# XiangpengHao/pq-vector

Measured on AMD Instinct MI355X. Metric: topk_queries_per_s_k10, higher is better.
Workload: dtype f32

## Files before the change

pq-vector_amd/csrc/api.cpp:

```cpp
#include "../../include/pqv.h"

#include <hip/hip_runtime.h>
#include <time.h>
#include <unistd.h>

#include <algorithm>
#include <atomic>
#include <functional>
#include <system_error>
#include <thread>
#include <cmath>
#include <chrono>
#include <cstdio>
#include <cstdlib>
#include <cstring>
#include <condition_variable>
#include <memory>
#include <mutex>
#include <new>
#include <string>
#include <type_traits>
#include <unordered_map>
#include <unordered_set>
#include <vector>
// ... 271 lines not shown
    }
};

constexpr int PQV_LANES = 4;
struct Scratch {
    DevBuf s_probe_keys, s_probe_vals, s_probe, s_cand_base, s_ncand, s_part_keys, s_part_vals, s_queries, s_rows,
        s_dist, s_nfound, s_pair_u32, s_pairs, s_groups, s_quads, s_items, s_ticket, s_ticket2, s_cand_keys, s_cand_vals, s_cand_cnt, s_spilled,
        s_seed_ub, s_qblk, s_gthr, s_tie, s_replay, s_qnorm, s_qmax, s_thr_hist, s_thr_bins, s_qi8, s_qn2i, s_qres, s_qresu, s_pair_lb, s_part_flags, s_qpad, s_cand_lb, s_pendv, s_work, s_nwork, s_out,
        s_hit_cnt, s_hit_keys, s_hit_vals, s_alt_keys, s_alt_vals, s_rsegs, s_rout_off, s_rout_rows, s_rout_dist,
        s_pair_end, s_file_cnt,
        s_qcos,
        s_qkeys,
        s_qfilt_a, s_qfilt_b,
        s_part_grp, s_grp_out,
        s_g1_rows, s_g1_dist, s_g1_keys, s_g1_nfound, s_gset_keys, s_gset_slot, s_gpart_slot, s_gpart_cnt, s_grows_out,
        s_expand_cnt, s_expand_used;
    PinnedBuf h_io;
    hipEvent_t done = nullptr;
    hipStream_t stream = nullptr;
    bool used = false;
    hipStream_t side = nullptr;
    hipEvent_t ev_fork = nullptr, ev_join = nullptr;
    std::vector<const DevBuf *> bufs() const {
        return {&s_probe_keys, &s_probe_vals, &s_probe, &s_cand_base, &s_ncand, &s_part_keys, &s_part_vals, &s_queries, &s_rows,
                &s_dist, &s_nfound, &s_pair_u32, &s_pairs, &s_groups, &s_quads, &s_items, &s_ticket, &s_ticket2, &s_cand_keys, &s_cand_vals, &s_cand_cnt, &s_spilled,
                &s_seed_ub, &s_qblk, &s_gthr, &s_tie, &s_replay, &s_qnorm, &s_qmax, &s_thr_hist, &s_thr_bins, &s_qi8, &s_qn2i, &s_qres, &s_qresu, &s_pair_lb, &s_part_flags, &s_qpad, &s_cand_lb, &s_pendv, &s_work, &s_nwork, &s_out,
                &s_hit_cnt, &s_hit_keys, &s_hit_vals, &s_alt_keys, &s_alt_vals, &s_rsegs, &s_rout_off, &s_rout_rows, &s_rout_dist,
                &s_pair_end, &s_file_cnt, &s_qcos, &s_qkeys, &s_qfilt_a, &s_qfilt_b, &s_part_grp, &s_grp_out,
                &s_g1_rows, &s_g1_dist, &s_g1_keys, &s_g1_nfound, &s_gset_keys, &s_gset_slot, &s_gpart_slot, &s_gpart_cnt, &s_grows_out,
                &s_expand_cnt, &s_expand_used};
    }
    ~Scratch() {
        if (done) (void)hipEventDestroy(done);
        if (ev_fork) (void)hipEventDestroy(ev_fork);
        if (ev_join) (void)hipEventDestroy(ev_join);
        if (side) (void)hipStreamDestroy(side);
    }
};

struct pqv_searcher {
    int device = 0;
    uint64_t uid = 0;
    uint32_t dim = 0, n_clusters = 0;
    uint32_t sdim = 0;
    uint64_t n = 0;
    uint64_t max_list_len = 0;
    pqv_corpus *corpus = nullptr;
    std::vector<uint64_t> h_list_off;
    std::shared_ptr<ListRows> h_rows;
    DevBuf d_cent_t;
    uint32_t kc_pad = 0;
    DevBuf d_centroids, d_list_off, d_ids, d_mat_ivf, d_stats;
    mutable DevBuf d_row_norm2;
    const float *d_mat = nullptr;
    const uint32_t *d_row_of = nullptr;
    const uint32_t *d_final_ids = nullptr;
    bool images_only = false;
    hipStream_t stream = nullptr;
    mutable std::mutex mu;
    mutable Scratch lanes[PQV_LANES];
    mutable PinnedBuf h_wide_stats;
    mutable uint32_t lane_rr = 0;
    mutable DevBuf d_mat_blk_op[3], d_blk_off;
    mutable bool f16_ok = false;
    mutable float f16_scale = 1.0f;
    mutable bool norms_done = false;
// ... 10 lines not shown
        uint32_t cand_cap = 0;
        int screen_f16 = 1;
        int screen_i8 = 1;
        uint32_t seed_rows = 0;
        uint32_t wide_rows = 0;
        uint32_t tile_rows = 0;
        int running_thr = 1;
        int defer = 1;
        int quad_xcd = -1;
        int single_bucket = 1;
        int seed_refine = 1;
        int item_grid = 1;
        int chunk_major = 1;
        int wide_waves = 0;
        int probe_rows = 1;
        uint32_t quad_width = 0;
        uint32_t min_blocks = 0;
        int pair_prune = 1;
        int i8_form = 0;
        int xcd_items = 1;
        int pf96 = 1;
        int drain_min = 0;
        int fork_wide = 0;
        int wide_quads = 1;
        uint32_t wide_quad_rows = 0;
        int list_once = 0;
    };
    mutable Opts opt;
    uint32_t n_files = 0;
    std::vector<uint32_t> seg_off;
    std::vector<uint64_t> row_base;
    uint32_t seg_max_kc = 0;
    bool rr_cap = false;
    DevBuf d_seg_off, d_seg_off64;
    mutable pqv_counters_t counters{};
    mutable bool timing = false;
    mutable std::vector<hipEvent_t> ev;
    mutable std::unique_ptr<pqv_corpus> cos_corpus;
    mutable std::unique_ptr<pqv_searcher> cos;
    ~pqv_searcher();
};
pqv_searcher::~pqv_searcher() {
    for (auto e : ev) (void)hipEventDestroy(e);
    pool_put(device, stream);
}

static int lane_acquire(const pqv_searcher *s, hipStream_t stream, Scratch **out) {
    Scratch *sc = nullptr;
    for (auto &l : s->lanes) if (l.used && l.stream == stream) { sc = &l; break; }
    if (!sc) for (auto &l : s->lanes) if (!l.used) { sc = &l; break; }
    if (!sc) sc = &s->lanes[s->lane_rr++ % PQV_LANES];
    if (!sc->done) HIP_TRY(hipEventCreateWithFlags(&sc->done, hipEventDisableTiming));
    if (sc->used && sc->stream != stream) HIP_TRY(hipStreamWaitEvent(stream, sc->done, 0));
    sc->stream = stream; sc->used = true;
    *out = sc;
    return PQV_OK;
}
// ... 2556 lines not shown
    o.cand_cap = static_cast<uint32_t>(std::max<long long>(0, num("PQV_CAND_CAP", o.cand_cap)));
    o.screen_f16 = num("PQV_SCREEN_F16", o.screen_f16) != 0;
    o.screen_i8 = static_cast<int>(num("PQV_SCREEN_I8", o.screen_i8));
    o.seed_rows = static_cast<uint32_t>(num("PQV_SEED_ROWS", o.seed_rows));
    o.wide_rows = static_cast<uint32_t>(num("PQV_WIDE_ROWS", o.wide_rows));
    o.tile_rows = static_cast<uint32_t>(num("PQV_TILE_ROWS", o.tile_rows));
    o.running_thr = num("PQV_RUNNING_THR", o.running_thr) != 0;
    o.defer = static_cast<int>(num("PQV_DEFER", o.defer));
    o.quad_xcd = static_cast<int>(num("PQV_QUAD_XCD", o.quad_xcd));
    o.wide_waves = static_cast<int>(num("PQV_WIDE_WAVES", o.wide_waves));
    o.item_grid = static_cast<int>(num("PQV_ITEM_GRID", o.item_grid));
    o.chunk_major = static_cast<int>(num("PQV_CHUNK_MAJOR", o.chunk_major));
    o.seed_refine = static_cast<int>(num("PQV_SEED_REFINE", o.seed_refine));
    o.single_bucket = static_cast<int>(num("PQV_SINGLE_BUCKET", o.single_bucket));
    o.probe_rows = static_cast<int>(num("PQV_PROBE_ROWS", o.probe_rows));
    o.quad_width = static_cast<uint32_t>(num("PQV_QUAD_WIDTH", o.quad_width));
    o.min_blocks = static_cast<uint32_t>(num("PQV_MIN_BLOCKS", o.min_blocks));
    o.wide_quads = static_cast<int>(num("PQV_WIDE_QUADS", o.wide_quads));
    o.fork_wide = static_cast<int>(num("PQV_FORK_WIDE", o.fork_wide));
    o.drain_min = static_cast<int>(num("PQV_DRAIN_MIN", o.drain_min));
    o.pf96 = static_cast<int>(num("PQV_PF96", o.pf96));
    o.xcd_items = static_cast<int>(num("PQV_XCD_ITEMS", o.xcd_items));
    o.wide_quad_rows = static_cast<uint32_t>(num("PQV_WIDE_QUAD_ROWS", o.wide_quad_rows));
    o.list_once = static_cast<int>(num("PQV_LIST_ONCE", o.list_once));
    o.pair_prune = static_cast<int>(num("PQV_PAIR_PRUNE", o.pair_prune));
    o.i8_form = static_cast<int>(num("PQV_I8_FORM", o.i8_form));
}

bool wide_rows_nt(const pqv_searcher *s) {
    if (!s->h_wide_stats.p) return true;
// ... 135 lines not shown
        HIP_TRY(hipStreamSynchronize(stream));
    } else if (op == 1) {
        HIP_TRY(blk.alloc(tiles * 16 * s->sdim * 2));
        HIP_TRY(launch_block_rows_f16(s->d_mat, s->d_list_off.as<uint64_t>(), s->d_blk_off.as<uint64_t>(), kc,
                                      (s->max_list_len + 15) / 16, s->sdim, s->f16_scale, blk.p, stream, s->d_row_of));
    } else {
        HIP_TRY(blk.alloc(tiles * 16 * s->sdim * sizeof(float)));
        HIP_TRY(launch_block_rows(s->d_mat, s->d_list_off.as<uint64_t>(), s->d_blk_off.as<uint64_t>(), kc,
                                  (s->max_list_len + 15) / 16, s->sdim, blk.p, stream, s->d_row_of));
    }
    HIP_TRY(hipStreamSynchronize(stream));
    undo.done = true;
    return PQV_OK;
}

}

static int pqv_searcher_create_impl(const pqv_index *index, pqv_corpus *corpus, uint32_t flags,
                                   pqv_searcher **out) {
    if (!out) return fail(PQV_ERR_INVALID, "out must not be NULL");
    *out = nullptr;
    const auto t_enter = std::chrono::steady_clock::now();
    if (!index || !corpus) return fail(PQV_ERR_INVALID, "index/corpus must not be NULL");
    if (index->dim != corpus->dim)
        return fail(PQV_ERR_INVALID, "index dimension " + std::to_string(index->dim) +
                                         " does not match corpus dimension " + std::to_string(corpus->dim));
    if (index->permutation_of != 0 ? index->permutation_of != corpus->n : false)
        return fail(PQV_ERR_INVALID, "index row id out of range for this corpus");
    uint64_t known_bound = 0;
    if (index->permutation_of == 0 && !(index->known_row_bound(&known_bound) && known_bound <= corpus->n)) {
// ... 40 lines not shown
    mark("validation + host copies");
    S_TRY(pool_get(s->device, &s->stream));
    mark("stream");
    S_TRY(s->d_centroids.alloc(index->centroids.size() * sizeof(float)));
    S_TRY(s->d_list_off.alloc(index->list_off.size() * sizeof(uint64_t)));
    S_TRY(s->d_ids.alloc(std::max<size_t>(1, s->n) * sizeof(uint32_t)));
    mark("allocations");
    S_TRY(hipMemcpyAsync(s->d_centroids.p, index->centroids.data(), index->centroids.size() * sizeof(float),
                         hipMemcpyHostToDevice, s->stream));
    S_TRY(hipMemcpyAsync(s->d_list_off.p, index->list_off.data(), index->list_off.size() * sizeof(uint64_t),
                         hipMemcpyHostToDevice, s->stream));
    if ((s->dim % 4) == 0 && s->n_clusters) {
        s->kc_pad = (s->n_clusters + 255) / 256 * 256;
        S_TRY(s->d_cent_t.alloc(static_cast<size_t>(s->kc_pad) * s->dim * sizeof(float)));
        S_TRY(pqv::launch_transpose_rows4(s->d_centroids.as<float>(), s->n_clusters, s->kc_pad, s->dim, s->d_cent_t.p, s->stream));
    }
    mark("centroid tables");
    if (s->n) {
        const DevRows *dr = index->rows->dev.get();
        if (dr && dr->p && dr->device == s->device && dr->n == s->n) {
            S_TRY(hipMemcpyAsync(s->d_ids.p, dr->p, s->n * sizeof(uint32_t), hipMemcpyDeviceToDevice, s->stream));
        } else {
            const std::vector<uint32_t> *rv = index->rows->get();
            if (!rv) { delete s; return PQV_ERR_HIP; }
            S_TRY(hipMemcpyAsync(s->d_ids.p, rv->data(), s->n * sizeof(uint32_t), hipMemcpyHostToDevice, s->stream));
        }
    }
    mark("tables + ids upload");
    {
        const char *e = std::getenv("PQV_IVF_COPY");
// ... 283 lines not shown
    }
}

void stream_split(uint64_t max_len, uint64_t pairs, uint32_t &rows_per_block, uint32_t &blocks_per_list) {
    const uint64_t bpl = std::max<uint64_t>(1, std::min<uint64_t>((8192 + pairs - 1) / pairs, (max_len + 255) / 256));
    const uint64_t rpb = ((max_len + bpl - 1) / bpl + 255) / 256 * 256;
    rows_per_block = static_cast<uint32_t>(rpb);
    blocks_per_list = static_cast<uint32_t>((max_len + rpb - 1) / rpb);
}

struct TopkPlan {
    uint32_t np;
    uint32_t probe_bpl;
    uint32_t probe_kpart;
    bool probe_rows;
    uint32_t rr_rows_per_block, rr_bpl;
    uint32_t n_part_probe, n_part_rr;
    bool tile;
    uint32_t max_groups;
    bool filter;
    uint32_t seed_rows, filter_bpl;
    bool f16;
    bool i8;
    bool quad;
    uint32_t filter_rows_per_block, max_quads, quad_width;
    uint32_t block_waves;
    uint32_t slots_per_pair;
    uint32_t wide_width;
    uint32_t wide_rows_per_block, wide_bpl;
    bool list_once;
// ... 14 lines not shown
}
static bool seed_refine_on(const pqv_searcher *s, uint32_t nq, uint32_t k) {
    (void)nq;
    return s->opt.seed_refine && (!s->d_row_of || s->images_only) && (s->sdim % 32) == 0 && k <= 16 && (s->opt.seed_refine > 1 || s->sdim >= 256);
}
TopkPlan plan_topk(const pqv_searcher *s, uint32_t nq, uint32_t nprobe, uint32_t k = 1, int metric = 0, bool exact_stream = false) {
    TopkPlan p{};
    const pqv_searcher::Opts &o = s->opt;
    if (metric == PQV_DOT) exact_stream = true;
    p.np = probe_count(s, nprobe);
    p.probe_bpl = (s->n_clusters + 255) / 256;
    p.n_part_probe = p.probe_bpl * pqv::waves_per_block();
    p.probe_rows = s->opt.probe_rows && s->kc_pad != 0 && (nq >= 8 || s->opt.probe_rows > 1) &&
                   static_cast<uint64_t>(nq) * s->kc_pad * 12 <= (2ull << 30);
    if (metric == PQV_DOT) p.probe_rows = false;
    p.probe_kpart = p.probe_rows ? 64u : p.np;
    if (s->n_files && !p.probe_rows) {
        p.probe_bpl = (s->seg_max_kc + 255) / 256;
        p.n_part_probe = s->n_files * p.probe_bpl * pqv::waves_per_block();
        p.probe_kpart = std::min<uint32_t>(nprobe, s->seg_max_kc);
    }
    const uint64_t max_len = std::max<uint64_t>(1, s->max_list_len);
    const uint64_t pairs = std::max<uint64_t>(1, static_cast<uint64_t>(nq) * p.np);
    p.tile = metric == PQV_L2SQ_REF4 && k <= 256 && pairs >= 4ull * s->n_clusters;
    const uint64_t mean_len = s->n / std::max<uint32_t>(1, s->n_clusters);
    const bool wide_ok = o.filter_variant == 0 && wide_path_possible(s);
    const bool wide_any_batch = metric == PQV_L2SQ_REF4 && o.tile_filter && k <= 128 && wide_ok && mean_len >= 192;
    if (wide_any_batch) p.tile = true;
    if (o.rerank_mode == 1) p.tile = false;
    if (o.rerank_mode == 2) p.tile = metric == PQV_L2SQ_REF4 && k <= 256;
// ... 115 lines not shown
    pm.part_keys = sc.s_probe_keys.as<uint64_t>(); pm.part_vals = sc.s_probe_vals.as<uint32_t>();
    pm.nq = nq; pm.n_part = p.n_part_probe; pm.k_part = p.probe_kpart; pm.k = p.np;
    pm.list_off = s->d_list_off.as<uint64_t>();
    pm.probe = sc.s_probe.as<uint32_t>(); pm.cand_base = sc.s_cand_base.as<uint64_t>();
    pm.n_cand = sc.s_ncand.as<uint64_t>();
    pm.max_pos = max_candidates ? max_candidates : ~0ull;
    return PQV_OK;
}

int enqueue_probe(const pqv_searcher *s, Scratch &sc, const TopkPlan &p, const float *d_queries, uint32_t nq, uint32_t nprobe,
                  uint64_t max_candidates, const pqv::MergeArgs &pm, uint32_t *zero_u32, uint32_t zero_n, hipStream_t stream,
                  int metric = PQV_L2SQ_REF4) {
    using namespace pqv;
    uint64_t *keys = const_cast<uint64_t *>(pm.part_keys);
    uint32_t *vals = const_cast<uint32_t *>(pm.part_vals);
    if (p.probe_rows) {
        ProbeRowsArgs pr{};
        pr.cent_t = s->d_cent_t.as<float4>(); pr.queries = d_queries;
        pr.nq = nq; pr.kc = s->n_clusters; pr.kc_pad = s->kc_pad; pr.dim = s->dim;
        pr.part_keys = keys; pr.part_vals = vals;
        pr.zero_u32 = zero_u32; pr.zero_n = zero_n;
        HIP_TRY(launch_probe_rows(pr, stream));
    } else {
        StreamArgs pa{};
        pa.mat = s->d_centroids.as<float>();
        if (s->n_files) {
            HIP_TRY(launch_seg_probe_fill(s->d_seg_off.as<uint32_t>(), s->n_files, nq, sc.s_probe.as<uint32_t>(), sc.s_cand_base.as<uint64_t>(), stream));
            pa.list_off = s->d_seg_off64.as<uint64_t>(); pa.probe = sc.s_probe.as<uint32_t>(); pa.cand_base = sc.s_cand_base.as<uint64_t>();
            pa.nprobe = s->n_files;
        } else {
            pa.single_begin = 0; pa.single_end = s->n_clusters;
// ... 2030 lines not shown
    else if (n == "cand_cap") o.cand_cap = static_cast<uint32_t>(std::max<int64_t>(0, value));
    else if (n == "screen_f16") o.screen_f16 = value != 0;
    else if (n == "screen_i8") o.screen_i8 = static_cast<int>(value);
    else if (n == "seed_rows") o.seed_rows = static_cast<uint32_t>(std::max<int64_t>(0, value));
    else if (n == "wide_rows") o.wide_rows = static_cast<uint32_t>(std::max<int64_t>(0, value));
    else if (n == "tile_rows") o.tile_rows = static_cast<uint32_t>(std::max<int64_t>(0, value));
    else if (n == "running_thr") o.running_thr = value != 0;
    else if (n == "defer") o.defer = static_cast<int>(value);
    else if (n == "quad_xcd") o.quad_xcd = static_cast<int>(value);
    else if (n == "wide_waves") o.wide_waves = static_cast<int>(value);
    else if (n == "single_bucket") o.single_bucket = static_cast<int>(value);
    else if (n == "seed_refine") o.seed_refine = static_cast<int>(value);
    else if (n == "item_grid") o.item_grid = static_cast<int>(value);
    else if (n == "chunk_major") o.chunk_major = value != 0;
    else if (n == "probe_rows") o.probe_rows = static_cast<int>(value);
    else if (n == "quad_width") o.quad_width = static_cast<uint32_t>(std::max<int64_t>(0, value));
    else if (n == "min_blocks") o.min_blocks = static_cast<uint32_t>(std::max<int64_t>(0, value));
    else if (n == "pair_prune") o.pair_prune = value != 0;
    else if (n == "wide_quads") o.wide_quads = value <= 0 ? 0 : value >= 2 ? 2 : 1;
    else if (n == "fork_wide") o.fork_wide = value <= 0 ? 0 : value >= 2 ? 2 : 1;
    else if (n == "pf96") o.pf96 = value <= 0 ? 0 : value >= 2 ? 2 : 1;
    else if (n == "drain_min") o.drain_min = static_cast<int>(std::max<int64_t>(0, std::min<int64_t>(64, value)));
    else if (n == "xcd_items") o.xcd_items = static_cast<int>(std::max<int64_t>(0, std::min<int64_t>(3, value)));
    else if (n == "wide_quad_rows") o.wide_quad_rows = static_cast<uint32_t>(std::max<int64_t>(0, value));
    else if (n == "list_once") o.list_once = static_cast<int>(value);
    else if (n == "i8_form") {
        o.i8_form = static_cast<int>(std::min<int64_t>(2, std::max<int64_t>(0, value)));
        (void)hipSetDevice(s->device);
        (void)hipDeviceSynchronize();
        s->d_mat_blk_op[2].release();
// ... 93 lines not shown
                      defp ? "true" : "false", seed_ng, qlds ? "true" : "false", op, rt.seed_tail ? 12 : 1, S,
                      std::max<uint32_t>(1, nq) * (seed_refine_on(s, std::max<uint32_t>(1, nq), k) ? 256u : 64u));
        if (p.wide_width) {
            const size_t l = std::strlen(kn);
            if (p.list_once) std::snprintf(kn + l, sizeof kn - l, "; list_filter_kernel<%u, %d>", s->sdim / 64, S);
            else
            std::snprintf(kn + l, sizeof kn - l, "; wide_filter_kernel<%u, 8, %d, true, 2, false, %s, 2, %s>", p.wide_width / 16, S, wide_rows_nt(s) ? "true" : "false",
                          defp ? "true" : "false");
        }
    }
    if (metric == PQV_DOT) {
        const bool al = (s->sdim % 4) == 0;
        std::snprintf(kn, sizeof kn, " | kernels: dot_stream_kernel<%d, %d, 0, %s, 0>; dot_merge_kernel<%d>",
                      (al && (s->sdim / 4) % 64 == 0) ? 64 : 32, k <= 64 ? 1 : k <= 256 ? 4 : 16, al ? "true" : "false", k <= 64 ? 1 : k <= 256 ? 4 : 16);
    }
    std::snprintf(buf, len, "%s%s; centroid probe: %s%s", tb, t, p.probe_rows ? "probe_rows_kernel (a lane per centroid)" : metric == PQV_DOT ? "dot_stream_kernel" : "stream_kernel", kn);
    return PQV_OK;
}
extern "C" int pqv_searcher_describe(const pqv_searcher *s, uint32_t nq, uint32_t k, uint32_t nprobe, int metric,
                                     char *buf, size_t len) {
    return guard([&] { return pqv_searcher_describe_impl(s, nq, k, nprobe, metric, buf, len); });
}

static int pqv_searcher_footprint_impl(const pqv_searcher *s, uint64_t *row_order_bytes, uint64_t *ivf_rows_bytes,
                                       uint64_t *blocked_bytes, uint64_t *other_bytes) {
    if (!s) return fail(PQV_ERR_INVALID, "searcher must not be NULL");
    std::lock_guard<std::mutex> lock(s->mu);
    if (row_order_bytes) *row_order_bytes = s->corpus && s->corpus->d_rows ? s->corpus->capacity * s->corpus->dim * sizeof(float) : 0;
    if (ivf_rows_bytes) *ivf_rows_bytes = s->d_mat_ivf.p ? s->d_mat_ivf.bytes : 0;
    if (blocked_bytes) *blocked_bytes = (s->d_mat_blk_op[0].p ? s->d_mat_blk_op[0].bytes : 0) + (s->d_mat_blk_op[1].p ? s->d_mat_blk_op[1].bytes : 0) +
                                        (s->d_mat_blk_op[2].p ? s->d_mat_blk_op[2].bytes : 0);
    uint64_t other = s->d_centroids.bytes + s->d_cent_t.bytes + s->d_list_off.bytes + s->d_ids.bytes + s->d_stats.bytes + s->d_row_norm2.bytes + s->d_blk_off.bytes +
                     s->d_center.bytes + s->d_list_scale.bytes + s->d_list_half.bytes + s->d_list_radius.bytes + s->d_row_n2i.bytes + s->d_row_res.bytes;
    for (const Scratch &l : s->lanes)
        for (const DevBuf *b : l.bufs()) other += b->p ? b->bytes : 0;
    if (other_bytes) *other_bytes = other;
    if (s->cos) {
        uint64_t f[4] = {0, 0, 0, 0};
        if (int rc = pqv_searcher_footprint_impl(s->cos.get(), f, f + 1, f + 2, f + 3)) return rc;
        if (row_order_bytes) *row_order_bytes += f[0];
        if (ivf_rows_bytes) *ivf_rows_bytes += f[1];
        if (blocked_bytes) *blocked_bytes += f[2];
        if (other_bytes) *other_bytes += f[3];
    }
    return PQV_OK;
}
extern "C" int pqv_searcher_footprint(const pqv_searcher *s, uint64_t *row_order_bytes, uint64_t *ivf_rows_bytes,
// ... 729 lines not shown
```

pq-vector_amd/csrc/kernels.h:

```cpp
#pragma once
#include <hip/hip_runtime.h>
#include <stdint.h>

namespace pqv {

constexpr uint64_t KEY_EMPTY = ~0ull;

enum StreamMode : int {
    STREAM_TOPK   = 0,
    STREAM_DIST   = 1,
    STREAM_MINUPD = 2,
    STREAM_RANGE  = 3,
};

struct StreamArgs {
    const float    *mat;
    const uint32_t *row_of;
    const uint64_t *list_off;
    const uint32_t *probe;
    const uint64_t *cand_base;
    uint64_t        single_begin, single_end;
    const float    *queries;
    uint32_t        nq, nprobe, dim, k;
    uint32_t        rows_per_block;
// ... 191 lines not shown
hipError_t launch_predicate_rows(const PredArgs &a, hipStream_t s);
hipError_t launch_mask_gather(const uint64_t *rowbits, uint64_t n_rows, const uint32_t *ids, uint64_t n_pos, uint64_t *bits,
                              uint64_t n_words, unsigned long long *count, hipStream_t s);
hipError_t launch_mask_pack(const uint8_t *allowed, uint64_t n_rows, uint64_t *rowbits, uint64_t n_words, hipStream_t s);

struct ProbeRowsArgs {
    const float4   *cent_t;
    const float    *queries;
    uint32_t        nq, kc, kc_pad, dim;
    uint64_t       *part_keys;
    uint32_t       *part_vals;
    uint32_t       *zero_u32;
    uint32_t        zero_n;
};
hipError_t launch_probe_rows(const ProbeRowsArgs &a, hipStream_t s);
struct MergeArgs;
struct PairQuantArgs;
hipError_t launch_probe_single(const ProbeRowsArgs &pr, const MergeArgs &a, uint32_t *ticket, const PairQuantArgs *quant, hipStream_t s);
hipError_t launch_transpose_rows4(const float *rows, uint32_t kc, uint32_t kc_pad, uint32_t dim, void *out, hipStream_t s);

struct PairQuantArgs {
    const float    *queries;
    const uint32_t *probe;
    const float    *center;
    const float    *scale;
    const float    *half;
    const float    *radius;
    uint32_t        n_pairs, nprobe, dim;
    int8_t         *q_i8;
    int            *q_n2i;
// ... 284 lines not shown
    float           kA;
    float           eps, cm;
    uint32_t       *cand;
    float          *cand_t;
    uint32_t       *cand_cnt;
    float          *best_t;
    uint32_t        cap;
};
hipError_t launch_assign_wide(const AssignWideArgs &a, hipStream_t s);
hipError_t launch_assign_resolve(const AssignWideArgs &a, const float *rows, const float *centroids, uint32_t dim, uint32_t *cluster,
                                 unsigned long long *stats , hipStream_t s);
hipError_t launch_assign_rescore(const float *rows, const float *centroids, uint64_t m, uint32_t dim, uint32_t kc, const uint32_t *cand,
                                 const uint32_t *cand_cnt, uint32_t cap, uint32_t *cluster, hipStream_t s);
hipError_t launch_center_normalize_f16(const float *rows, const float *mu, uint64_t n, uint64_t n_pad, uint32_t dim, uint32_t dim_p,
                                       float *out_n2, void *out, hipStream_t s, float fixed_scale = 0.0f, const uint32_t *idx = nullptr);
hipError_t launch_col_mean(const float *m, uint32_t k, uint32_t dim, float *mu, hipStream_t s);
hipError_t launch_normalize_f16(const float *rows, const float *rnorm, uint64_t n, uint32_t dim, uint32_t dim_p, void *out, hipStream_t s);
hipError_t launch_normalize_i8(const float *rows, const float *rnorm, uint64_t n, uint32_t dim, uint32_t dim_p, void *out, void *sr, float *nrm,
                               float *maxima , hipStream_t s);
hipError_t launch_brute_rescore(const BruteArgs &a, const uint32_t *first, hipStream_t s);
hipError_t launch_row_norms(const float *rows, uint64_t n, uint32_t dim, int mode, float *out, hipStream_t s);
hipError_t launch_brute_select(unsigned long long *cand, uint32_t *cand_cnt, uint32_t cap, uint32_t nq,
                               uint32_t k, unsigned long long *thr, uint32_t *overflow, hipStream_t s);
hipError_t launch_brute_overflow_check(const uint32_t *cand_cnt, uint32_t nq, uint32_t cap, uint32_t *overflow,
                                       hipStream_t s);
hipError_t launch_brute_finish(const unsigned long long *cand, const uint32_t *cand_cnt, uint32_t cap,
                               uint32_t nq, uint32_t k, uint32_t *row_idx, float *dist, uint32_t *n_found,
                               hipStream_t s);

hipError_t launch_shard_merge(const float *dist, const uint32_t *rows, const long long *row_base,
// ... 153 lines not shown
```

pq-vector_amd/csrc/kernels_all.hip:

```cpp
#include "kernels_probe.hip"
#include "kernels_screen.hip"
#include "kernels_brute.hip"
#include "kernels_build.hip"
#include "kernels_layout.hip"
#include "kernels_list.hip"
#include "kernels_kpp.hip"
#include "kernels_range.hip"
#include "kernels_mask.hip"
#include "kernels_predicate.hip"
#include "kernels_distinct.hip"
#include "kernels_grouped.hip"
#include "kernels_dot.hip"
#include "kernels_expand.hip"
#include "kernels_distinct_filter.hip"
#include "kernels_group_expand.hip"
#include "kernels_append.hip"
#include "kernels_remove.hip"
```

pq-vector_amd/csrc/kernels_build.hip:

```cpp
#include "device_common.hpp"

namespace pqv {

__global__ __launch_bounds__(256, 2) void assign_f16_kernel(const AssignF16Args a) {
    __shared__ float4 As4[2][BH_BM * 4];
    __shared__ float4 Bs4[2][BH_BN * 4];
    __shared__ uint32_t thr_s[BH_BM];
    __shared__ float xn2_s[BH_BM];

    const int tid = threadIdx.x, lane = tid & 63, wave = tid >> 6;
    const int wm = wave >> 1, wn = wave & 1;
    const uint64_t m0 = (uint64_t)blockIdx.x * BH_BM;
    const uint32_t dp = a.dim_p;
    const int ld_r = tid >> 2, ld_ch = tid & 3;
    float4 ra[2], rb[4];
    const uint64_t qleft = (a.m - m0) * dp * 2;
    const __amdgpu_buffer_rsrc_t qres = __builtin_amdgcn_make_buffer_rsrc(
        const_cast<uint16_t *>(a.x16 + m0 * dp), 0, (int)(qleft > 0xFFFFFFFFull ? 0xFFFFFFFFu : (uint32_t)qleft), 0x00020000);
    const uint32_t lane_b = (uint32_t)ld_r * dp * 2 + (uint32_t)ld_ch * 16, r64_b = 64u * dp * 2;
    __shared__ float xs_s[BH_BM];
    if (tid < BH_BM) {
        thr_s[tid] = 0x7F800000u;
        const float xn = m0 + tid < a.m ? a.xn2[m0 + tid] : 0.0f;
        xn2_s[tid] = xn;
// ... 719 lines not shown
            v = fminf(fmaxf(v, -65504.0f), 65504.0f);
            const _Float16 h = (_Float16)v;
            out[r * dim_p + e] = __builtin_bit_cast(uint16_t, h);
        }
    }
}
hipError_t launch_center_normalize_f16(const float *rows, const float *mu, uint64_t n, uint64_t n_pad, uint32_t dim, uint32_t dim_p,
                                       float *out_n2, void *out, hipStream_t s, float fixed_scale, const uint32_t *idx) {
    if (n_pad == 0) return hipSuccess;
    uint64_t blocks = (n_pad + 3) / 4;
    if (blocks > 65536) blocks = 65536;
    hipLaunchKernelGGL(center_normalize_f16_kernel, dim3((uint32_t)blocks), dim3(256), 0, s, rows, mu, n, n_pad, dim, dim_p, out_n2,
                       static_cast<uint16_t *>(out), fixed_scale, idx);
    return hipGetLastError();
}
__global__ __launch_bounds__(1024) void col_mean_kernel(const float *__restrict__ m, uint32_t k, uint32_t dim, float *__restrict__ mu) {
    __shared__ float part[16][64];
    const uint32_t lane = threadIdx.x & 63u, d = blockIdx.x * 64u + lane, sl = threadIdx.x >> 6;
    float acc = 0.0f;
    if (d < dim) {
        uint32_t r = sl;
        for (; r + 48 < k; r += 64) {
            const float v0 = m[(uint64_t)r * dim + d], v1 = m[(uint64_t)(r + 16) * dim + d];
            const float v2 = m[(uint64_t)(r + 32) * dim + d], v3 = m[(uint64_t)(r + 48) * dim + d];
            acc += (v0 + v1) + (v2 + v3);
        }
        for (; r < k; r += 16) acc += m[(uint64_t)r * dim + d];
    }
    part[sl][lane] = acc;
    __syncthreads();
// ... 355 lines not shown
```

Measured before the change: 606,300.

## Screen IVF centroid probe with f16 MFMA bounds, exact distances only for contenders

Adds a two-kernel centroid probe path. An f16 MFMA GEMM scores mean-centred, scaled queries against centroids, then derives rigorous lower and upper distance bounds from an error model. A resolve kernel picks the nprobe-th upper bound as a threshold and computes exact fp32 distances only for centroids whose lower bound does not exceed it. This replaces the full fp32 probe_rows computation when enough queries and clusters are present. It adds centroid preprocessing at searcher creation and extra scratch memory, and falls back to evaluating every centroid exactly when the candidate list overflows.

Result: faster. 621,400 (median of 6 runs) (+2.5%).

```diff
diff --git a/pq-vector_amd/csrc/api.cpp b/pq-vector_amd/csrc/api.cpp
--- a/pq-vector_amd/csrc/api.cpp
+++ b/pq-vector_amd/csrc/api.cpp
@@ -309,7 +309,8 @@
         s_qfilt_a, s_qfilt_b,
         s_part_grp, s_grp_out,
         s_g1_rows, s_g1_dist, s_g1_keys, s_g1_nfound, s_gset_keys, s_gset_slot, s_gpart_slot, s_gpart_cnt, s_grows_out,
-        s_expand_cnt, s_expand_used;
+        s_expand_cnt, s_expand_used,
+        s_ps_q16, s_ps_qn2, s_ps_score;
     PinnedBuf h_io;
     hipEvent_t done = nullptr;
     hipStream_t stream = nullptr;
@@ -323,7 +324,7 @@
                 &s_hit_cnt, &s_hit_keys, &s_hit_vals, &s_alt_keys, &s_alt_vals, &s_rsegs, &s_rout_off, &s_rout_rows, &s_rout_dist,
                 &s_pair_end, &s_file_cnt, &s_qcos, &s_qkeys, &s_qfilt_a, &s_qfilt_b, &s_part_grp, &s_grp_out,
                 &s_g1_rows, &s_g1_dist, &s_g1_keys, &s_g1_nfound, &s_gset_keys, &s_gset_slot, &s_gpart_slot, &s_gpart_cnt, &s_grows_out,
-                &s_expand_cnt, &s_expand_used};
+                &s_expand_cnt, &s_expand_used, &s_ps_q16, &s_ps_qn2, &s_ps_score};
     }
     ~Scratch() {
         if (done) (void)hipEventDestroy(done);
@@ -345,6 +346,9 @@
     std::shared_ptr<ListRows> h_rows;
     DevBuf d_cent_t;
     uint32_t kc_pad = 0;
+    DevBuf d_ps_mu, d_ps_c16, d_ps_cn2;
+    mutable DevBuf d_ps_stats;
+    struct ProbeScreen { bool ok = false, tried = false; uint32_t dim_p = 0; float inv_cs = 0, fn = 0, e1 = 0, e2s = 0, kS = 0, lo_f = 0, hi_f = 0; } ps;
     DevBuf d_centroids, d_list_off, d_ids, d_mat_ivf, d_stats;
     mutable DevBuf d_row_norm2;
     const float *d_mat = nullptr;
@@ -385,6 +389,7 @@
         int chunk_major = 1;
         int wide_waves = 0;
         int probe_rows = 1;
+        int probe_screen = 1;
         uint32_t quad_width = 0;
         uint32_t min_blocks = 0;
         int pair_prune = 1;
@@ -412,6 +417,12 @@
     ~pqv_searcher();
 };
 pqv_searcher::~pqv_searcher() {
+    if (d_ps_stats.p) {
+        unsigned long long h[3] = {0, 0, 0};
+        if (hipDeviceSynchronize() == hipSuccess && hipMemcpy(h, d_ps_stats.p, sizeof h, hipMemcpyDeviceToHost) == hipSuccess)
+            std::fprintf(stderr, "[pqv] screened probe: %llu queries, %.2f exact evaluations per query of %u centroids, %llu all-exact queries\n",
+                         h[0], h[0] ? static_cast<double>(h[1]) / static_cast<double>(h[0]) : 0.0, n_clusters, h[2]);
+    }
     for (auto e : ev) (void)hipEventDestroy(e);
     pool_put(device, stream);
 }
@@ -2998,6 +3009,7 @@
     o.seed_refine = static_cast<int>(num("PQV_SEED_REFINE", o.seed_refine));
     o.single_bucket = static_cast<int>(num("PQV_SINGLE_BUCKET", o.single_bucket));
     o.probe_rows = static_cast<int>(num("PQV_PROBE_ROWS", o.probe_rows));
+    o.probe_screen = static_cast<int>(num("PQV_PROBE_SCREEN", o.probe_screen));
     o.quad_width = static_cast<uint32_t>(num("PQV_QUAD_WIDTH", o.quad_width));
     o.min_blocks = static_cast<uint32_t>(num("PQV_MIN_BLOCKS", o.min_blocks));
     o.wide_quads = static_cast<int>(num("PQV_WIDE_QUADS", o.wide_quads));
@@ -3163,6 +3175,47 @@
     return PQV_OK;
 }
 
+hipError_t probe_screen_images(pqv_searcher *s) {
+    using namespace pqv;
+    const uint32_t kc = s->n_clusters, dim = s->dim, dim_p = (dim + 63) / 64 * 64;
+    s->ps.tried = true;
+#define PS_TRY(expr) do { hipError_t _e = (expr); if (_e != hipSuccess) return _e; } while (0)
+    PS_TRY(s->d_ps_mu.alloc(static_cast<size_t>(dim) * sizeof(float)));
+    PS_TRY(s->d_ps_c16.alloc(static_cast<size_t>(s->kc_pad) * dim_p * sizeof(uint16_t)));
+    PS_TRY(s->d_ps_cn2.alloc(static_cast<size_t>(s->kc_pad) * sizeof(float)));
+    const float *d_c = s->d_centroids.as<float>();
+    PS_TRY(launch_col_mean(d_c, kc, dim, s->d_ps_mu.as<float>(), s->stream));
+    PS_TRY(launch_center_normalize_f16(d_c, s->d_ps_mu.as<float>(), kc, s->kc_pad, dim, dim_p, s->d_ps_cn2.as<float>(), s->d_ps_c16.p, s->stream));
+    std::vector<float> h_cn2(kc);
+    PS_TRY(hipMemcpyAsync(h_cn2.data(), s->d_ps_cn2.p, static_cast<size_t>(kc) * sizeof(float), hipMemcpyDeviceToHost, s->stream));
+    PS_TRY(hipStreamSynchronize(s->stream));
+    double mx = 0.0;
+    for (float v : h_cn2) { if (!(v <= 3.0e38f)) return hipSuccess; mx = std::max<double>(mx, v); }
+    const float cscale = mx > 0.0 ? static_cast<float>(256.0 / (std::sqrt(mx) * 1.000001)) : 1.0f;
+    const float inv_cs = static_cast<float>(1.000001 / static_cast<double>(cscale));
+    if (!(cscale > 0.0f && cscale < 3.0e38f && inv_cs > 0.0f && inv_cs < 3.0e38f)) return hipSuccess;
+    PS_TRY(launch_center_normalize_f16(d_c, s->d_ps_mu.as<float>(), kc, s->kc_pad, dim, dim_p, s->d_ps_cn2.as<float>(), s->d_ps_c16.p, s->stream, cscale));
+#undef PS_TRY
+    const double u = 5.9604644775390625e-08, h = 4.8828125e-04, hp = h + u + h * u;
+    const double sub = std::sqrt(static_cast<double>(dim)) * 2.98023223876953125e-08;
+    const double g = (center_normalize_f16_sum_depth(dim) + 2) * u * 1.01;
+    const double cm = (dim / 4 + 8) * u;
+    auto up = [](double v) { return std::nextafter(static_cast<float>(v), INFINITY); };
+    pqv_searcher::ProbeScreen &ps = s->ps;
+    ps.dim_p = dim_p; ps.inv_cs = inv_cs;
+    ps.fn = up((1.0 + g) * 1.000001);
+    ps.e1 = up((2.0 * hp + hp * hp + 1.01 * 2.02 * dim_p * u + 1.01 * sub / 256.0 + 2.0e-6) * 1.001);
+    ps.e2s = up(static_cast<double>(inv_cs) * sub * 1.02);
+    ps.kS = up(1.01 * g + 16.0 * u);
+    ps.lo_f = std::nextafter(static_cast<float>(1.0 - cm - 1.0e-6), 0.0f);
+    ps.hi_f = up(1.0 + cm + 1.0e-6);
+    ps.ok = ps.e2s < 3.0e38f;
+    if (const char *e = std::getenv("PQV_PROBE_SCREEN_STATS"); e && *e && *e != '0') {
+        if (s->d_ps_stats.alloc(3 * sizeof(unsigned long long)) == hipSuccess) (void)hipMemsetAsync(s->d_ps_stats.p, 0, 3 * sizeof(unsigned long long), s->stream);
+    }
+    return hipSuccess;
+}
+
 }
 
 static int pqv_searcher_create_impl(const pqv_index *index, pqv_corpus *corpus, uint32_t flags,
@@ -3233,6 +3286,9 @@
         s->kc_pad = (s->n_clusters + 255) / 256 * 256;
         S_TRY(s->d_cent_t.alloc(static_cast<size_t>(s->kc_pad) * s->dim * sizeof(float)));
         S_TRY(pqv::launch_transpose_rows4(s->d_centroids.as<float>(), s->n_clusters, s->kc_pad, s->dim, s->d_cent_t.p, s->stream));
+        if (s->opt.probe_screen) {
+            if (hipError_t e = probe_screen_images(s)) S_TRY(e);
+        }
     }
     mark("centroid tables");
     if (s->n) {
@@ -3546,6 +3602,7 @@
     uint32_t probe_bpl;
     uint32_t probe_kpart;
     bool probe_rows;
+    bool probe_screen;
     uint32_t rr_rows_per_block, rr_bpl;
     uint32_t n_part_probe, n_part_rr;
     bool tile;
@@ -3590,6 +3647,8 @@
     p.probe_rows = s->opt.probe_rows && s->kc_pad != 0 && (nq >= 8 || s->opt.probe_rows > 1) &&
                    static_cast<uint64_t>(nq) * s->kc_pad * 12 <= (2ull << 30);
     if (metric == PQV_DOT) p.probe_rows = false;
+    p.probe_screen = p.probe_rows && s->ps.ok && o.probe_screen && !s->n_files && p.np >= 1 && p.np <= s->n_clusters / 4 &&
+                     (o.probe_screen > 1 || (nq >= 128 && s->n_clusters >= 256));
     p.probe_kpart = p.probe_rows ? 64u : p.np;
     if (s->n_files && !p.probe_rows) {
         p.probe_bpl = (s->seg_max_kc + 255) / 256;
@@ -3735,7 +3794,23 @@
     using namespace pqv;
     uint64_t *keys = const_cast<uint64_t *>(pm.part_keys);
     uint32_t *vals = const_cast<uint32_t *>(pm.part_vals);
-    if (p.probe_rows) {
+    if (p.probe_screen) {
+        const pqv_searcher::ProbeScreen &ps = s->ps;
+        HIP_TRY(sc.s_ps_q16.ensure(static_cast<size_t>(nq) * ps.dim_p * sizeof(uint16_t)));
+        HIP_TRY(sc.s_ps_qn2.ensure(static_cast<size_t>(nq) * sizeof(float)));
+        HIP_TRY(sc.s_ps_score.ensure(static_cast<size_t>(nq) * s->kc_pad * sizeof(float)));
+        HIP_TRY(launch_center_normalize_f16(d_queries, s->d_ps_mu.as<float>(), nq, nq, s->dim, ps.dim_p, sc.s_ps_qn2.as<float>(), sc.s_ps_q16.p, stream));
+        ProbeScreenArgs pr{};
+        pr.q16 = sc.s_ps_q16.as<uint16_t>(); pr.c16 = s->d_ps_c16.as<uint16_t>(); pr.qn2 = sc.s_ps_qn2.as<float>(); pr.cn2 = s->d_ps_cn2.as<float>();
+        pr.score = sc.s_ps_score.as<float>(); pr.queries = d_queries; pr.centroids = s->d_centroids.as<float>();
+        pr.nq = nq; pr.kc = s->n_clusters; pr.kc_pad = s->kc_pad; pr.dim = s->dim; pr.dim_p = ps.dim_p; pr.np = p.np;
+        pr.inv_cs = ps.inv_cs; pr.fn = ps.fn; pr.e1 = ps.e1; pr.e2s = ps.e2s; pr.kS = ps.kS; pr.lo_f = ps.lo_f; pr.hi_f = ps.hi_f;
+        pr.part_keys = keys; pr.part_vals = vals;
+        pr.zero_u32 = zero_u32; pr.zero_n = zero_n;
+        pr.stats = s->d_ps_stats.as<unsigned long long>();
+        HIP_TRY(launch_probe_screen(pr, stream));
+        s->counters.kernel_launches += 2;
+    } else if (p.probe_rows) {
         ProbeRowsArgs pr{};
         pr.cent_t = s->d_cent_t.as<float4>(); pr.queries = d_queries;
         pr.nq = nq; pr.kc = s->n_clusters; pr.kc_pad = s->kc_pad; pr.dim = s->dim;
@@ -5796,6 +5871,13 @@
     else if (n == "item_grid") o.item_grid = static_cast<int>(value);
     else if (n == "chunk_major") o.chunk_major = value != 0;
     else if (n == "probe_rows") o.probe_rows = static_cast<int>(value);
+    else if (n == "probe_screen") {
+        o.probe_screen = static_cast<int>(value);
+        if (value != 0 && !s->ps.tried && s->kc_pad != 0 && !s->n_files) {
+            const hipError_t e = probe_screen_images(s);
+            if (e != hipSuccess) return fail(e == hipErrorOutOfMemory ? PQV_ERR_OOM : PQV_ERR_HIP, std::string("probe_screen_images: ") + hipGetErrorString(e));
+        }
+    }
     else if (n == "quad_width") o.quad_width = static_cast<uint32_t>(std::max<int64_t>(0, value));
     else if (n == "min_blocks") o.min_blocks = static_cast<uint32_t>(std::max<int64_t>(0, value));
     else if (n == "pair_prune") o.pair_prune = value != 0;
@@ -5919,7 +6001,8 @@
         std::snprintf(kn, sizeof kn, " | kernels: dot_stream_kernel<%d, %d, 0, %s, 0>; dot_merge_kernel<%d>",
                       (al && (s->sdim / 4) % 64 == 0) ? 64 : 32, k <= 64 ? 1 : k <= 256 ? 4 : 16, al ? "true" : "false", k <= 64 ? 1 : k <= 256 ? 4 : 16);
     }
-    std::snprintf(buf, len, "%s%s; centroid probe: %s%s", tb, t, p.probe_rows ? "probe_rows_kernel (a lane per centroid)" : metric == PQV_DOT ? "dot_stream_kernel" : "stream_kernel", kn);
+    std::snprintf(buf, len, "%s%s; centroid probe: %s%s", tb, t, p.probe_screen ? "probe_screen_kernel + probe_resolve_kernel (f16 contraction, probe_rows_kernel's exact chains for the contenders)"
+                  : p.probe_rows ? "probe_rows_kernel (a lane per centroid)" : metric == PQV_DOT ? "dot_stream_kernel" : "stream_kernel", kn);
     return PQV_OK;
 }
 extern "C" int pqv_searcher_describe(const pqv_searcher *s, uint32_t nq, uint32_t k, uint32_t nprobe, int metric,
@@ -5935,7 +6018,7 @@
     if (ivf_rows_bytes) *ivf_rows_bytes = s->d_mat_ivf.p ? s->d_mat_ivf.bytes : 0;
     if (blocked_bytes) *blocked_bytes = (s->d_mat_blk_op[0].p ? s->d_mat_blk_op[0].bytes : 0) + (s->d_mat_blk_op[1].p ? s->d_mat_blk_op[1].bytes : 0) +
                                         (s->d_mat_blk_op[2].p ? s->d_mat_blk_op[2].bytes : 0);
-    uint64_t other = s->d_centroids.bytes + s->d_cent_t.bytes + s->d_list_off.bytes + s->d_ids.bytes + s->d_stats.bytes + s->d_row_norm2.bytes + s->d_blk_off.bytes +
+    uint64_t other = s->d_centroids.bytes + s->d_cent_t.bytes + s->d_ps_mu.bytes + s->d_ps_c16.bytes + s->d_ps_cn2.bytes + s->d_ps_stats.bytes + s->d_list_off.bytes + s->d_ids.bytes + s->d_stats.bytes + s->d_row_norm2.bytes + s->d_blk_off.bytes +
                      s->d_center.bytes + s->d_list_scale.bytes + s->d_list_half.bytes + s->d_list_radius.bytes + s->d_row_n2i.bytes + s->d_row_res.bytes;
     for (const Scratch &l : s->lanes)
         for (const DevBuf *b : l.bufs()) other += b->p ? b->bytes : 0;
diff --git a/pq-vector_amd/csrc/kernels.h b/pq-vector_amd/csrc/kernels.h
--- a/pq-vector_amd/csrc/kernels.h
+++ b/pq-vector_amd/csrc/kernels.h
@@ -229,6 +229,26 @@
     uint32_t        zero_n;
 };
 hipError_t launch_probe_rows(const ProbeRowsArgs &a, hipStream_t s);
+struct ProbeScreenArgs {
+    const uint16_t *q16;
+    const uint16_t *c16;
+    const float    *qn2;
+    const float    *cn2;
+    float          *score;
+    const float    *queries;
+    const float    *centroids;
+    uint32_t        nq, kc, kc_pad, dim, dim_p, np;
+    float           inv_cs;
+    float           fn;
+    float           e1, e2s, kS;
+    float           lo_f, hi_f;
+    uint64_t       *part_keys;
+    uint32_t       *part_vals;
+    uint32_t       *zero_u32;
+    uint32_t        zero_n;
+    unsigned long long *stats;
+};
+hipError_t launch_probe_screen(const ProbeScreenArgs &a, hipStream_t s);
 struct MergeArgs;
 struct PairQuantArgs;
 hipError_t launch_probe_single(const ProbeRowsArgs &pr, const MergeArgs &a, uint32_t *ticket, const PairQuantArgs *quant, hipStream_t s);
@@ -543,6 +563,7 @@
                                  const uint32_t *cand_cnt, uint32_t cap, uint32_t *cluster, hipStream_t s);
 hipError_t launch_center_normalize_f16(const float *rows, const float *mu, uint64_t n, uint64_t n_pad, uint32_t dim, uint32_t dim_p,
                                        float *out_n2, void *out, hipStream_t s, float fixed_scale = 0.0f, const uint32_t *idx = nullptr);
+uint32_t center_normalize_f16_sum_depth(uint32_t dim);
 hipError_t launch_col_mean(const float *m, uint32_t k, uint32_t dim, float *mu, hipStream_t s);
 hipError_t launch_normalize_f16(const float *rows, const float *rnorm, uint64_t n, uint32_t dim, uint32_t dim_p, void *out, hipStream_t s);
 hipError_t launch_normalize_i8(const float *rows, const float *rnorm, uint64_t n, uint32_t dim, uint32_t dim_p, void *out, void *sr, float *nrm,
diff --git a/pq-vector_amd/csrc/kernels_all.hip b/pq-vector_amd/csrc/kernels_all.hip
--- a/pq-vector_amd/csrc/kernels_all.hip
+++ b/pq-vector_amd/csrc/kernels_all.hip
@@ -1,4 +1,5 @@
 #include "kernels_probe.hip"
+#include "kernels_probe_screen.hip"
 #include "kernels_screen.hip"
 #include "kernels_brute.hip"
 #include "kernels_build.hip"
diff --git a/pq-vector_amd/csrc/kernels_build.hip b/pq-vector_amd/csrc/kernels_build.hip
--- a/pq-vector_amd/csrc/kernels_build.hip
+++ b/pq-vector_amd/csrc/kernels_build.hip
@@ -757,6 +757,10 @@
                        static_cast<uint16_t *>(out), fixed_scale, idx);
     return hipGetLastError();
 }
+uint32_t center_normalize_f16_sum_depth(uint32_t dim) {
+    const uint32_t per_lane = ((dim & 7u) == 0 && dim <= 2048) ? 8u * ((dim / 8u + 63u) / 64u) : (dim + 63u) / 64u;
+    return per_lane + 6u;
+}
 __global__ __launch_bounds__(1024) void col_mean_kernel(const float *__restrict__ m, uint32_t k, uint32_t dim, float *__restrict__ mu) {
     __shared__ float part[16][64];
     const uint32_t lane = threadIdx.x & 63u, d = blockIdx.x * 64u + lane, sl = threadIdx.x >> 6;
diff --git a/pq-vector_amd/csrc/kernels_probe_screen.hip b/pq-vector_amd/csrc/kernels_probe_screen.hip
--- /dev/null
+++ b/pq-vector_amd/csrc/kernels_probe_screen.hip
@@ -0,0 +1,254 @@
+#include "device_common.hpp"
+
+namespace pqv {
+
+__global__ __launch_bounds__(256, 2) void probe_screen_kernel(const ProbeScreenArgs a) {
+    if (a.zero_u32 && blockIdx.x == 0) {
+        for (uint32_t i = blockIdx.y * 256 + threadIdx.x; i < a.zero_n; i += gridDim.y * 256) a.zero_u32[i] = 0u;
+    }
+    __shared__ float4 lds[4096];
+    const int lane = threadIdx.x & 63, wave = __builtin_amdgcn_readfirstlane(threadIdx.x >> 6);
+    const int l31 = lane & 31, lk = lane >> 5;
+    float4 *const As = lds + wave * 1024, *const Bs = As + 512;
+    auto sw = [](int r) { return ((r >> 1) & 1) | (((r >> 2) & 3) << 1); };
+    const uint32_t q0 = blockIdx.y * 64u, c0 = blockIdx.x * 64u;
+    const int ld_r = lane >> 3, ld_ch = lane & 7;
+    const uint32_t rowb = a.dim_p / 8u;
+    const float4 *const qb = reinterpret_cast<const float4 *>(a.q16) + (uint64_t)q0 * rowb + ld_ch;
+    const float4 *const cb = reinterpret_cast<const float4 *>(a.c16) + (uint64_t)(c0 + ld_r) * rowb + ld_ch;
+    uint32_t qo[8];
+#pragma unroll
+    for (int h = 0; h < 8; ++h) {
+        const uint32_t qr = q0 + ld_r + 8 * h < a.nq ? q0 + ld_r + 8 * h : a.nq - 1;
+        qo[h] = (qr - q0) * rowb;
+    }
+    const uint32_t nk = a.dim_p / 64u;
+    f32x16_t acc00, acc01, acc10, acc11;
+#pragma unroll
+    for (int r = 0; r < 16; ++r) { acc00[r] = 0.0f; acc01[r] = 0.0f; acc10[r] = 0.0f; acc11[r] = 0.0f; }
+    for (uint32_t kt = wave; kt < nk; kt += 4) {
+        float4 ra[8], rb[8];
+#pragma unroll
+        for (int h = 0; h < 8; ++h) { ra[h] = qb[qo[h] + kt * 8]; rb[h] = cb[(uint32_t)(8 * h) * rowb + kt * 8]; }
+#pragma unroll
+        for (int h = 0; h < 8; ++h) {
+            const int r = ld_r + 8 * h;
+            As[r * 8 + (ld_ch ^ sw(r))] = ra[h];
+            Bs[r * 8 + (ld_ch ^ sw(r))] = rb[h];
+        }
+#pragma unroll
+        for (int j = 0; j < 4; ++j) {
+            float4 av[2], bv[2];
+#pragma unroll
+            for (int t = 0; t < 2; ++t) {
+                const int r = t * 32 + l31;
+                av[t] = As[r * 8 + ((2 * j + lk) ^ sw(r))];
+                bv[t] = Bs[r * 8 + ((2 * j + lk) ^ sw(r))];
+            }
+            acc00 = __builtin_amdgcn_mfma_f32_32x32x16_f16(__builtin_bit_cast(f16x8_t, av[0]), __builtin_bit_cast(f16x8_t, bv[0]), acc00, 0, 0, 0);
+            acc01 = __builtin_amdgcn_mfma_f32_32x32x16_f16(__builtin_bit_cast(f16x8_t, av[0]), __builtin_bit_cast(f16x8_t, bv[1]), acc01, 0, 0, 0);
+            acc10 = __builtin_amdgcn_mfma_f32_32x32x16_f16(__builtin_bit_cast(f16x8_t, av[1]), __builtin_bit_cast(f16x8_t, bv[0]), acc10, 0, 0, 0);
+            acc11 = __builtin_amdgcn_mfma_f32_32x32x16_f16(__builtin_bit_cast(f16x8_t, av[1]), __builtin_bit_cast(f16x8_t, bv[1]), acc11, 0, 0, 0);
+        }
+    }
+    __syncthreads();
+    float *red = reinterpret_cast<float *>(lds);
+#pragma unroll
+    for (int r = 0; r < 16; ++r) {
+        red[((wave * 4 + 0) * 16 + r) * 64 + lane] = acc00[r];
+        red[((wave * 4 + 1) * 16 + r) * 64 + lane] = acc01[r];
+        red[((wave * 4 + 2) * 16 + r) * 64 + lane] = acc10[r];
+        red[((wave * 4 + 3) * 16 + r) * 64 + lane] = acc11[r];
+    }
+    __syncthreads();
+    const int tm = wave >> 1, tn = wave & 1;
+#pragma unroll
+    for (int r = 0; r < 16; ++r) {
+        const int o = ((tm * 2 + tn) * 16 + r) * 64 + lane;
+        const float v = (red[o] + red[4096 + o]) + (red[8192 + o] + red[12288 + o]);
+        const uint32_t q = q0 + (uint32_t)(tm * 32 + (r & 3) + 8 * (r >> 2) + 4 * lk);
+        if (q < a.nq) a.score[(uint64_t)q * a.kc_pad + c0 + (uint32_t)(tn * 32 + l31)] = v;
+    }
+}
+
+struct ProbeBound { float lb, ub; };
+__device__ __forceinline__ ProbeBound probe_bound(const ProbeScreenArgs &a, float an2, float an_ub, float bn2, float s) {
+    const float bn_ub = sqrtf(bn2) * a.fn;
+    const float est = s * (sqrtf(an2) * 0.00390625f) * a.inv_cs;
+    const float S = an2 + bn2;
+    const float mid = S - 2.0f * est;
+    const float E = (a.kS * S + 2.0f * an_ub * (bn_ub * a.e1 + a.e2s)) * 1.00001f + 1.0e-33f;
+    ProbeBound r;
+    const float lo = mid - E, hi = mid + E;
+    const bool finite = fabsf(S) < INFINITY && fabsf(est) < INFINITY && fabsf(mid) < INFINITY && E < INFINITY &&
+                        fabsf(lo) < INFINITY && hi < 3.0e38f;
+    r.lb = finite ? fmaxf(lo, 0.0f) * a.lo_f : 0.0f;
+    r.ub = finite ? fmaxf(hi, 0.0f) * a.hi_f + 1.0e-33f : INFINITY;
+    return r;
+}
+
+constexpr uint32_t PR_CAP = 2048;
+constexpr uint32_t PR_GS = 192;
+constexpr uint32_t PR_TW = PR_GS + 4;
+constexpr uint32_t PR_R = 32;
+
+__global__ __launch_bounds__(256) void probe_resolve_kernel(const ProbeScreenArgs a) {
+    __shared__ uint32_t s_hist[256];
+    __shared__ uint32_t s_sel[4];
+    __shared__ uint32_t s_list[PR_CAP];
+    __shared__ __attribute__((aligned(16))) float s_term[PR_R * PR_TW];
+    const uint32_t q = blockIdx.x;
+    const int lane = threadIdx.x & 63, wave = threadIdx.x >> 6;
+    const float an2 = a.qn2[q];
+    const float an_ub = sqrtf(an2) * a.fn;
+    const float *sc = a.score + (uint64_t)q * a.kc_pad;
+    uint64_t *pk = a.part_keys + (uint64_t)q * a.kc_pad;
+    uint32_t *pv = a.part_vals + (uint64_t)q * a.kc_pad;
+    bool all = !(an2 < INFINITY);
+    float Tf = INFINITY;
+    const bool parked = 2u * a.kc <= PR_R * PR_TW;
+    float *s_ub = s_term, *s_lb = s_term + a.kc;
+    auto bound = [&](uint32_t c) {
+        ProbeBound b = probe_bound(a, an2, an_ub, a.cn2[c], sc[c]);
+        if (!(b.ub < INFINITY)) b.ub = INFINITY;
+        return b;
+    };
+    auto ub_of = [&](uint32_t c) { return parked ? s_ub[c] : bound(c).ub; };
+    if (!all) {
+        if (threadIdx.x == 0) { s_sel[2] = 0x7F800000u; s_sel[3] = 0u; }
+        __syncthreads();
+        uint32_t mn = 0x7F800000u, mx = 0u;
+        for (uint32_t c = threadIdx.x; c < a.kc; c += 256) {
+            const ProbeBound b = bound(c);
+            if (parked) { s_ub[c] = b.ub; s_lb[c] = b.lb; }
+            if (b.ub < INFINITY) { const uint32_t u = __float_as_uint(b.ub); mn = u < mn ? u : mn; mx = u > mx ? u : mx; }
+        }
+#pragma unroll
+        for (int off = 32; off > 0; off >>= 1) {
+            const uint32_t on = (uint32_t)__shfl_xor((int)mn, off, 64), ox = (uint32_t)__shfl_xor((int)mx, off, 64);
+            mn = on < mn ? on : mn; mx = ox > mx ? ox : mx;
+        }
+        if (lane == 0) { atomicMin(&s_sel[2], mn); atomicMax(&s_sel[3], mx); }
+        __syncthreads();
+        const float fmn = __uint_as_float(s_sel[2]), fmx = __uint_as_float(s_sel[3]);
+        const float scale = fmx > fmn ? 4.0e9f / (fmx - fmn) : 0.0f;
+        auto key_of = [&](uint32_t c) {
+            const float ub = ub_of(c);
+            if (!(ub < INFINITY)) return 0xFFFFFFFFu;
+            const float kf = (ub - fmn) * scale;
+            return kf < 4.2e9f ? (uint32_t)kf : 0xFFFFFFFEu;
+        };
+        __syncthreads();
+        const uint32_t Tk = block_kth_u32(key_of, a.kc, a.np, s_hist, s_sel);
+        if (threadIdx.x == 0) s_sel[3] = Tk == 0xFFFFFFFFu ? 0x7F800000u : 0u;
+        __syncthreads();
+        if (Tk != 0xFFFFFFFFu) {
+            uint32_t tm = 0u;
+            for (uint32_t c = threadIdx.x; c < a.kc; c += 256)
+                if (key_of(c) <= Tk) { const uint32_t u = __float_as_uint(ub_of(c)); tm = u > tm ? u : tm; }
+#pragma unroll
+            for (int off = 32; off > 0; off >>= 1) { const uint32_t o = (uint32_t)__shfl_xor((int)tm, off, 64); tm = o > tm ? o : tm; }
+            if (lane == 0) atomicMax(&s_sel[3], tm);
+        }
+        __syncthreads();
+        Tf = __uint_as_float(s_sel[3]);
+        all = !(Tf < INFINITY);
+    }
+    __syncthreads();
+    if (threadIdx.x == 0) s_sel[2] = 0u;
+    __syncthreads();
+    for (uint32_t c = threadIdx.x; c < a.kc_pad; c += 256) {
+        bool keep = false;
+        if (c < a.kc && !all) {
+            const float lb = parked ? s_lb[c] : bound(c).lb;
+            keep = !(lb > Tf);
+        }
+        if (keep) {
+            const uint32_t slot = atomicAdd(&s_sel[2], 1u);
+            if (slot < PR_CAP) s_list[slot] = c;
+        } else {
+            pk[c] = KEY_EMPTY; pv[c] = 0xFFFFFFFFu;
+        }
+    }
+    __syncthreads();
+    uint32_t m = s_sel[2];
+    if (all || m > PR_CAP) { all = true; m = a.kc; }
+    if (a.stats && threadIdx.x == 0) {
+        atomicAdd(&a.stats[0], 1ull);
+        atomicAdd(&a.stats[1], (unsigned long long)m);
+        if (all) atomicAdd(&a.stats[2], 1ull);
+    }
+    const uint32_t G = a.dim >> 2;
+    const float4 *qg = reinterpret_cast<const float4 *>(a.queries + (uint64_t)q * a.dim);
+    for (uint32_t p0 = 0; p0 < m; p0 += PR_R) {
+        float run = 0.0f;
+        for (uint32_t gs0 = 0; gs0 < G; gs0 += PR_GS) {
+            float4 qv[3];
+#pragma unroll
+            for (int j = 0; j < 3; ++j) {
+                const uint32_t g = gs0 + (uint32_t)lane + 64u * (uint32_t)j;
+                qv[j] = qg[g < G ? g : G - 1];
+            }
+#pragma unroll
+            for (int half = 0; half < 2; ++half) {
+                float4 xv[4][3];
+#pragma unroll
+                for (int i = 0; i < 4; ++i) {
+                    const uint32_t pi = p0 + 4u * (uint32_t)(half * 4 + i) + (uint32_t)wave;
+                    if (pi < m) {
+                        const uint32_t c = all ? pi : s_list[pi];
+                        const float4 *xg = reinterpret_cast<const float4 *>(a.centroids + (uint64_t)c * a.dim);
+#pragma unroll
+                        for (int j = 0; j < 3; ++j) {
+                            const uint32_t g = gs0 + (uint32_t)lane + 64u * (uint32_t)j;
+                            xv[i][j] = xg[g < G ? g : G - 1];
+                        }
+                    } else {
+#pragma unroll
+                        for (int j = 0; j < 3; ++j) xv[i][j] = make_float4(0.f, 0.f, 0.f, 0.f);
+                    }
+                }
+#pragma unroll
+                for (int i = 0; i < 4; ++i)
+#pragma unroll
+                    for (int j = 0; j < 3; ++j) {
+                        const float d0 = qv[j].x - xv[i][j].x, d1 = qv[j].y - xv[i][j].y, d2 = qv[j].z - xv[i][j].z, d3 = qv[j].w - xv[i][j].w;
+                        float t = d0 * d0 + d1 * d1;
+                        t = t + d2 * d2;
+                        t = t + d3 * d3;
+                        s_term[((uint32_t)wave * 8u + (uint32_t)(half * 4 + i)) * PR_TW + (uint32_t)lane + 64u * (uint32_t)j] = t;
+                    }
+            }
+            __syncthreads();
+            if (lane < 8) {
+                const uint32_t n = G - gs0 < PR_GS ? G - gs0 : PR_GS;
+                const float *row = s_term + ((uint32_t)wave * 8u + (uint32_t)lane) * PR_TW;
+                uint32_t g = 0;
+#pragma unroll 4
+                for (; g + 4 <= n; g += 4) {
+                    const float4 t = *reinterpret_cast<const float4 *>(row + g);
+                    run = run + t.x; run = run + t.y; run = run + t.z; run = run + t.w;
+                }
+                for (; g < n; ++g) run = run + row[g];
+            }
+            __syncthreads();
+        }
+        if (lane < 8 && p0 + 4u * (uint32_t)lane + (uint32_t)wave < m) {
+            const uint32_t li = p0 + 4u * (uint32_t)lane + (uint32_t)wave;
+            const uint32_t c = all ? li : s_list[li];
+            pk[c] = ((uint64_t)__float_as_uint(run) << 32) | c;
+            pv[c] = c;
+        }
+    }
+}
+
+hipError_t launch_probe_screen(const ProbeScreenArgs &a, hipStream_t s) {
+    if (a.nq == 0 || a.kc == 0) return hipSuccess;
+    if ((a.dim % 4) != 0 || (a.dim_p % 64) != 0 || a.dim_p < a.dim || (a.kc_pad % 256) != 0 || a.kc_pad < a.kc || a.np == 0 || a.np > a.kc)
+        return hipErrorInvalidValue;
+    hipLaunchKernelGGL(probe_screen_kernel, dim3(a.kc_pad / 64, (a.nq + 63) / 64), dim3(256), 0, s, a);
+    hipLaunchKernelGGL(probe_resolve_kernel, dim3(a.nq), dim3(256), 0, s, a);
+    return hipGetLastError();
+}
+
+}
```
